# terminusdb-labs/parallel-hnsw

Measured on AMD Instinct MI355X. Metric: queries/sec at recall@10≥0.95 on 1M×768 f32, higher is better.
Workload: dtype f32

## Files before the change

### parallel_hnsw_amd/csrc/api.hip

```cpp
#include <hip/hip_runtime.h>

#include <algorithm>
#include <atomic>
#include <cmath>
#include <cstdarg>
#include <cstdio>
#include <cstring>
#include <new>
#include <stdexcept>
#include <vector>

#include "exact_slices.h"
#include "phnsw_internal.h"

static thread_local std::string g_err;

void ph_set_error(const char *fmt, ...) {
  char buf[1024];
  va_list ap;
  va_start(ap, fmt);
  vsnprintf(buf, sizeof(buf), fmt, ap);
  va_end(ap);
  g_err = buf;
}
// ... 614 lines not shown
    a.collect_k = c.collect_k;
    a.collect_flags = c.collect_flags;
    a.collect_ids = c.out_ids;
    a.collect_d = c.out_d;
    a.out_ids = nullptr;
    a.out_d = nullptr;
    a.filter_flags = 0u;
  }
}

uint32_t ph_default_ovf_cap(uint32_t ef) {
  if (const char *e = getenv("PHNSW_OVF_CAP"))
    if (atoi(e) > 0) return (uint32_t)atoi(e);
  return std::max<uint32_t>(8192u, ef * 64u);
}
static uint32_t default_ovf_cap(uint32_t ef) { return ph_default_ovf_cap(ef); }

static uint64_t two_launch_min() {
  const char *e = getenv("PHNSW_TWO_LAUNCH_MIN");
  return (e && atoll(e) > 0) ? (uint64_t)atoll(e) : (uint64_t)PH_TWO_LAUNCH_MIN;
}
static std::atomic<uint64_t> g_two_launch_count{0};
extern "C" uint64_t phnsw_debug_two_launch_count(void) { return g_two_launch_count.load(); }
extern "C" uint32_t phnsw_debug_last_search_chunks(const phnsw_index *ix) { return ix ? ix->ws[ix->ws_last].n_chunks : 0; }

extern "C" int phnsw_stream_create_beside(int device, void *other_stream, void **out_stream) try {
  if (!out_stream) {
    ph_set_error("phnsw_stream_create_beside: out_stream is NULL");
    return PHNSW_E_INVALID;
  }
  PH_HIP(hipSetDevice(device));
  hipStream_t st = nullptr;
  int rc = ph_stream_beside((hipStream_t)other_stream, &st);
  if (rc) return rc;
  *out_stream = (void *)st;
  return 0;
} catch (...) { return ph_caught(); }

static int attach_probes(phnsw_index *mix, const PhSearchCall &c, PhSearchArgs &a) {
  (void)mix, (void)c, (void)a;
#ifdef PH_CELL_PROBE
  {
    static unsigned long long *probe_dev = nullptr;
    if (!probe_dev) {
      PH_HIP(hipMalloc(&probe_dev, 12 * sizeof(unsigned long long)));
      PH_HIP(hipMemset(probe_dev, 0, 12 * sizeof(unsigned long long)));
// ... 89 lines not shown
  if (split) {
    g_two_launch_count++;
    rc = ph_workspace_order_ensure(ws, a.nq);
    for (uint32_t l = first_big; l < a.n_layers && !rc; l++)
      rc = ph_layer_anchor_pos(ix->store, mix->layers[l - 1]);
    if (rc) return rc;
    if (a.collect_k) {
      const size_t need = (size_t)nq * a.ef * 4u;
      if (ws.park_ids_bytes < need) {
        if (ws.park_ids) PH_HIP(hipFree(ws.park_ids));
        ws.park_ids = nullptr, ws.park_ids_bytes = 0;
        PH_HIP(hipMalloc(&ws.park_ids, need));
        ws.park_ids_bytes = need;
      }
      if (ws.park_d_bytes < need) {
        if (ws.park_d) PH_HIP(hipFree(ws.park_d));
        ws.park_d = nullptr, ws.park_d_bytes = 0;
        PH_HIP(hipMalloc(&ws.park_d, need));
        ws.park_d_bytes = need;
      }
      a.out_ids = ws.park_ids;
      a.out_d = ws.park_d;
    }
  }
  rc = attach_probes(mix, c, a);
  if (rc) return rc;
  rc = ph_search_begin(ws, stream);
  if (rc) return rc;
  bool kept_table = false;
  if (c.hint && T && !split) {
    rc = ph_build_table_prepare(mix, ws, a, *c.hint, T, stream, &kept_table);
    if (rc) return rc;
  }
  const uint64_t tmax = (T && !kept_table) ? ph_tiny_max_positions(ix, a.n_layers, a.ef) : 0;
  const uint64_t chunk = (tmax && nq > tmax) ? tmax : nq;
  for (uint64_t c0 = 0; c0 < nq; c0 += chunk) {
    PhSearchArgs b = a;
    const uint64_t cnt = std::min<uint64_t>(chunk, nq - c0);
    const bool last_chunk = c0 + cnt == nq;
    b.nq = (uint32_t)cnt;
    if (b.order) {
      b.order += c0;
    } else if (c0) {
      const uint32_t ostride = out_stride ? out_stride : b.ef;
      if (b.queries) b.queries += c0 * c.ldq;
      if (b.qids) b.qids += c0;
      if (b.exclude) b.exclude += c0;
      if (b.filter) b.filter += c0 * b.filter_stride;
      if (b.label_want) b.label_want += c0;
      if (b.out_ids) b.out_ids += c0 * ostride, b.out_d += c0 * ostride;
      if (b.collect_k) b.collect_ids += c0 * b.collect_k, b.collect_d += c0 * b.collect_k;
      b.out_len += c0;
      if (b.out_stats) b.out_stats += 2 * c0;
      b.status += c0;
      if (b.out_hit) b.out_hit += c0;
      b.first_node += (uint32_t)c0;
    }
    ws.n_chunks = (uint32_t)(c0 / chunk) + 1;
    PH_HIP(hipEventRecord(ws.evc, stream));
    if (c0) PH_HIP(hipMemsetAsync(ws.dtotals, 0, sizeof(unsigned long long) * 3 * PH_MAX_DISPATCH, stream));
    if (!kept_table) {
      rc = ph_tiny_prepare(ix, ws, b, T, stream);
      if (rc) return rc;
    }
    ws.d_tiny = b.tiny_layers != 0;
    PH_HIP(hipEventRecord(ws.evd[0], stream));
    if (!split) {
      b.launch_totals = ws.dtotals;
      b.launch_tab = ws.dtotals + 2 * PH_MAX_DISPATCH;
      rc = ph_search_launch(ix, ws, b, stream, last_chunk);
      if (rc) return rc;
      PH_HIP(hipEventRecord(ws.evd[1], stream));
      ws.n_dispatch = 1;
      ws.d_lo[0] = knn_mode ? b.n_layers - 1 : 0;
      ws.d_hi[0] = b.n_layers;
      continue;
    }
    const uint32_t Td = b.tiny_layers;
    const bool dense_first = Td && Td < b.n_layers && b.nq >= PH_DENSE_SPLIT_MIN && !getenv("PHNSW_NO_DENSE_SPLIT");
    if (dense_first) b.dense_flag = ws.tiny_member + b.tiny_n;
    uint32_t di = 0;
    uint32_t *const out_hit_final = b.out_hit;
    const uint32_t first_hi = dense_first ? Td : first_big;
    for (uint32_t lo = 0, hi = first_hi; lo < b.n_layers; lo = hi, hi = (lo == Td && dense_first && first_big > Td) ? first_big : hi + 1) {
      PhSearchArgs p = b;
// ... 649 lines not shown
```

### parallel_hnsw_amd/csrc/bruteforce.hip

```cpp
#include <hip/hip_runtime.h>

#include <algorithm>
#include <vector>

#include "phnsw_device.h"

typedef float f32x16 __attribute__((ext_vector_type(16)));

#define BF_TM 128
#define BF_TN 128
#define BF_TK 32
#define BF_LD 132

__global__ __launch_bounds__(256) void ph_gemm_nt_mfma_kernel(const float *__restrict__ Q, uint32_t ldq, uint32_t nq,
                                                              const float *__restrict__ B, uint32_t ldb, uint32_t nb,
                                                              uint32_t K, float *__restrict__ C, uint64_t ldc) {
  __shared__ float Qs[BF_TK][BF_LD];
  __shared__ float Bs[BF_TK][BF_LD];
  const uint32_t t = threadIdx.x, lane = t & 63, w = t >> 6;
  const uint32_t wm = w >> 1, wn = w & 1;
  const uint32_t q0 = blockIdx.y * BF_TM, b0 = blockIdx.x * BF_TN;
  f32x16 acc[2][2];
#pragma unroll
  for (int i = 0; i < 2; i++)
#pragma unroll
// ... 250 lines not shown
    }
    __syncthreads();
    if (t == 0) {
      float b = -PH_FMAX;
      uint32_t i = PH_EMPTY32;
      for (int k = 0; k < 16; k++)
        if (widx[k] != PH_EMPTY32 && (i == PH_EMPTY32 || wbest[k] > b || (wbest[k] == b && widx[k] < i))) {
          b = wbest[k];
          i = widx[k];
        }
      cur_s = i;
      seen[i] = 1;
      rank[i] = step;
    }
    __syncthreads();
  }
}

__global__ void ph_rank_of_cell_kernel(uint32_t *pos, uint32_t n, const uint32_t *rank) {
  uint32_t i = blockIdx.x * blockDim.x + threadIdx.x;
  if (i < n) pos[i] = rank[pos[i]];
}

static int ph_store_anchors(phnsw_store *s) {
  if (s->anchors) return 0;
  uint32_t amax = 4096u;
  if (const char *e = getenv("PHNSW_ANCHORS")) amax = atoi(e) >= 64 ? (uint32_t)atoi(e) : amax;
  const uint32_t A = (uint32_t)std::min<uint64_t>(amax, std::max<uint64_t>(s->n / 16u, 1u)), ld = s->ld;
  const uint64_t stride = s->n / A;
  float *anchors = nullptr, *gram = nullptr;
  uint32_t *rank = nullptr, *ids = nullptr;
  std::vector<uint32_t> h(A);
  for (uint32_t a = 0; a < A; a++) h[a] = (uint32_t)(a * stride);
  hipError_t e = hipMalloc(&anchors, (size_t)A * ld * 4);
  if (e == hipSuccess) e = hipMalloc(&gram, (size_t)A * A * 4);
  if (e == hipSuccess) e = hipMalloc(&rank, (size_t)A * 4);
  if (e == hipSuccess) e = hipMalloc(&ids, (size_t)A * 4);
  if (e == hipSuccess) e = hipMemcpy(ids, h.data(), (size_t)A * 4, hipMemcpyHostToDevice);
  if (e == hipSuccess) {
    if (ph_store_converted(s))
      (void)ph_converted_gather_rows(s, ids, 0, A, anchors);
    else
      hipLaunchKernelGGL(ph_gather_rows_f32_kernel, dim3((A + 3) / 4), dim3(256), 0, 0, s->rows, ld, ids, 1u, A, anchors);
    dim3 grid((A + BF_TN - 1) / BF_TN, (A + BF_TM - 1) / BF_TM);
    hipLaunchKernelGGL(ph_gemm_nt_mfma_kernel, grid, dim3(256), 0, 0, anchors, ld, A, anchors, ld, A, ld, gram, (uint64_t)A);
    hipLaunchKernelGGL(ph_anchor_chain_kernel, dim3(1), dim3(1024), (A + 32) * 4, 0, gram, A, rank);
    e = hipGetLastError();
    if (e == hipSuccess) e = hipDeviceSynchronize();
  }
  if (gram) hipFree(gram);
  if (ids) hipFree(ids);
  if (e != hipSuccess) {
    if (anchors) hipFree(anchors);
    if (rank) hipFree(rank);
    return ph_hip_fail(e, "store cells (anchors)", __FILE__, __LINE__);
  }
  s->anchors = anchors;
  s->anchor_rank = rank;
  s->n_anchors = A;
  return 0;
}

void ph_store_anchors_free(phnsw_store *s) {
  if (s->anchors) hipFree(s->anchors);
  if (s->anchor_rank) hipFree(s->anchor_rank);
  s->anchors = nullptr;
  s->anchor_rank = nullptr;
}

bool ph_layer_wants_cells(const phnsw_store *s, uint32_t n_nodes) {
  return n_nodes >= PH_POS_MIN && (ph_store_f32(s) || ph_store_converted(s)) && s->n >= 65536 && s->metric != PHNSW_METRIC_L2 && !getenv("PHNSW_NO_LOCALITY");
}

int ph_layer_cells_range(const phnsw_store *cs, const PhLayerHost &L, uint32_t first, uint32_t count, uint32_t *out_pos) {
  phnsw_store *s = const_cast<phnsw_store *>(cs);
  if (count == 0) return 0;
  int rc = ph_store_anchors(s);
  if (rc) return rc;
  const uint32_t A = s->n_anchors, ld = s->ld;
  const uint32_t QC = 65536;
  float *qrows = nullptr, *scores = nullptr;
  hipError_t e = hipMalloc(&scores, (size_t)std::min(QC, count) * A * 4);
  if (e == hipSuccess && (!L.identity || ph_store_converted(s))) e = hipMalloc(&qrows, (size_t)std::min(QC, count) * ld * 4);
  if (e == hipSuccess) {
    for (uint32_t at = 0; at < count; at += QC) {
      const uint32_t cnt = std::min(QC, count - at);
      const float *Q = ph_store_f32(s) ? s->rows + (uint64_t)(first + at) * ld : nullptr;
      if (ph_store_converted(s)) {
        (void)ph_converted_gather_rows(s, L.identity ? nullptr : L.nodes + first + at, first + at, cnt, qrows);
        Q = qrows;
      } else if (!L.identity) {
        hipLaunchKernelGGL(ph_gather_rows_f32_kernel, dim3((cnt + 3) / 4), dim3(256), 0, 0, s->rows, ld, L.nodes + first + at,
                           1u, cnt, qrows);
        Q = qrows;
      }
      dim3 grid((A + BF_TN - 1) / BF_TN, (cnt + BF_TM - 1) / BF_TM);
      hipLaunchKernelGGL(ph_gemm_nt_mfma_kernel, grid, dim3(256), 0, 0, Q, ld, cnt, s->anchors, ld, A,
                         std::min<uint32_t>(ld, 256u), scores, (uint64_t)A);
      hipLaunchKernelGGL(ph_argmax_rows_kernel, dim3(std::min<uint32_t>(cnt, 256u * 16u)), dim3(64), 0, 0, scores,
                         (uint64_t)A, A, cnt, out_pos + at);
    }
    hipLaunchKernelGGL(ph_rank_of_cell_kernel, dim3((count + 255) / 256), dim3(256), 0, 0, out_pos, count, s->anchor_rank);
    e = hipGetLastError();
    if (e == hipSuccess) e = hipDeviceSynchronize();
  }
  if (e != hipSuccess) rc = ph_hip_fail(e, "layer cells (anchor GEMM)", __FILE__, __LINE__);
  if (qrows) hipFree(qrows);
  if (scores) hipFree(scores);
  return rc;
}

int ph_layer_anchor_pos(const phnsw_store *cs, PhLayerHost &L) {
  const uint32_t n = L.n_nodes;
  if (L.pos || !ph_layer_wants_cells(cs, n)) return 0;
  hipError_t e = hipMalloc(&L.pos, (size_t)n * 4);
  if (e != hipSuccess) return ph_hip_fail(e, "layer cells", __FILE__, __LINE__);
  int rc = ph_layer_cells_range(cs, L, 0, n, L.pos);
  if (rc) {
    hipFree(L.pos);
    L.pos = nullptr;
  }
  return rc;
}

extern "C" float phnsw_bruteforce_last_gemm_ms(void) { return g_bf_gemm_ms; }

extern "C" int phnsw_bruteforce_topk(const phnsw_store *s, const float *queries, uint64_t nq, uint32_t k,
                                     uint64_t *out_ids, float *out_d) try {
  if (int rc = ph_search_only_unsupported(s, "phnsw_bruteforce_topk")) return rc;
  if (!s || !queries || !out_ids || !out_d || nq == 0) {
    ph_set_error("phnsw_bruteforce_topk: invalid argument");
    return PHNSW_E_INVALID;
  }
  PH_HIP(hipSetDevice(s->device));
  float *qd = nullptr, *od = nullptr;
  uint32_t *oid = nullptr;
  hipError_t e = hipMalloc(&qd, (size_t)nq * s->ld * 4);
  if (e == hipSuccess && s->ld != s->dim) e = hipMemset(qd, 0, (size_t)nq * s->ld * 4);
  if (e == hipSuccess)
    e = hipMemcpy2D(qd, (size_t)s->ld * 4, queries, (size_t)s->dim * 4, (size_t)s->dim * 4, nq, hipMemcpyHostToDevice);
  if (e == hipSuccess) e = hipMalloc(&oid, (size_t)nq * k * 4);
  if (e == hipSuccess) e = hipMalloc(&od, (size_t)nq * k * 4);
  int rc = e == hipSuccess ? 0 : ph_hip_fail(e, "bruteforce staging", __FILE__, __LINE__);
  if (!rc) rc = phnsw_bruteforce_topk_device(s, qd, s->ld, nq, k, oid, od, nullptr);
  if (!rc) {
    std::vector<uint32_t> h((size_t)nq * k);
// ... 13 lines not shown
```

### parallel_hnsw_amd/csrc/build.hip

```cpp
#include <hip/hip_runtime.h>

#include <algorithm>
#include <cmath>
#include <cstdio>
#include <cstdlib>
#include <cstring>
#include <numeric>
#include <vector>

#include "phnsw_device.h"

int ph_sort_u32_host(uint32_t *keys, uint32_t n);
int ph_exclusive_scan_u32(const uint32_t *cnt, uint32_t n_plus_1, uint32_t *start, hipStream_t st);


template <typename T>
struct DevBuf {
  T *p = nullptr;
  size_t n = 0;
  int alloc(size_t count) {
    n = count;
    hipError_t e = ph_pool_alloc((void **)&p, std::max<size_t>(count, 1) * sizeof(T));
    if (e != hipSuccess) {
      p = nullptr;
// ... 1136 lines not shown
      }
      nodes[o++] = vecs[b++];
    }
  }
  std::vector<uint32_t> nb((size_t)n_new * W, PH_EMPTY32);
  std::vector<float> nd((size_t)n_new * W, PH_FMAX);
  for (uint32_t i = 0; i < n_old; i++)
    for (uint32_t k = 0; k < W; k++) {
      uint32_t x = old_nb[(size_t)i * W + k];
      nb[(size_t)old_map[i] * W + k] = x == PH_EMPTY32 ? PH_EMPTY32 : old_map[x];
      if (!old_d.empty()) nd[(size_t)old_map[i] * W + k] = old_d[(size_t)i * W + k];
    }
  PhLayerHost NL;
  PH_TRY(ph_layer_upload(ix, nodes.data(), nb.data(), n_new, W, &NL));
  if (!old_d.empty()) {
    hipError_t e = hipMalloc(&NL.nbr_dist, nd.size() * 4);
    if (e == hipSuccess) e = hipMemcpy(NL.nbr_dist, nd.data(), nd.size() * 4, hipMemcpyHostToDevice);
    if (e != hipSuccess) {
      ph_layer_free(NL);
      return ph_hip_fail(e, "extend_layer upload", __FILE__, __LINE__);
    }
  }
  if (L.pos) {
    std::vector<uint32_t> op(n_old), np(n_new, PH_EMPTY32);
    PH_HIP(hipMemcpy(op.data(), L.pos, (size_t)n_old * 4, hipMemcpyDeviceToHost));
    for (uint32_t i = 0; i < n_old; i++) np[old_map[i]] = op[i];
    uint32_t next = n_old;
    for (uint32_t i = 0; i < n_new; i++)
      if (np[i] == PH_EMPTY32) np[i] = next++;
    hipError_t e = hipMalloc(&NL.pos, (size_t)n_new * 4);
    if (e == hipSuccess) e = hipMemcpy(NL.pos, np.data(), (size_t)n_new * 4, hipMemcpyHostToDevice);
    if (e != hipSuccess) {
      ph_layer_free(NL);
      return ph_hip_fail(e, "extend_layer positions", __FILE__, __LINE__);
    }
  }
  ph_layer_free(L);
  ix->layers[lft] = NL;
  return 0;
}

__global__ void ph_gather_rows_kernel(const uint32_t *neighbors, uint32_t W, const uint32_t *which, uint32_t cnt,
                                      uint32_t *out) {
  uint64_t i = (uint64_t)blockIdx.x * blockDim.x + threadIdx.x;
  if (i >= (uint64_t)cnt * W) return;
  out[i] = neighbors[(size_t)which[i / W] * W + (i % W)];
}

static int filter_promotion_candidates_impl(phnsw_index *ix, uint32_t lft, const std::vector<uint32_t> &vecs,
                                            const phnsw_search_params *sp, std::vector<uint32_t> &sel) {
  sel.clear();
  if (lft == 0) return 0;
// ... 479 lines not shown
```

### parallel_hnsw_amd/csrc/group.hip

```cpp
#include <hip/hip_runtime.h>
#include <hipcub/hipcub.hpp>

#include "phnsw_internal.h"

#include "phnsw_device.h"

__global__ void ph_group_keys_kernel(const uint32_t *init_ids, const float *init_d, const uint32_t *init_len,
                                     uint32_t K, uint32_t n, uint64_t *keys, uint32_t *vals) {
  uint32_t i = blockIdx.x * blockDim.x + threadIdx.x;
  if (i >= n) return;
  bool some = init_len[i] != 0;
  uint32_t key = some ? init_ids[(size_t)i * K] : PH_EMPTY32;
  float d = some ? init_d[(size_t)i * K] : 0.f;
  keys[i] = ((uint64_t)key << 32) | fkey(d);
  vals[i] = i;
}

__global__ void ph_group_bounds_kernel(const uint64_t *keys, uint32_t n, uint32_t *gstart, uint32_t *gsize) {
  uint32_t p = blockIdx.x * blockDim.x + threadIdx.x;
  if (p >= n) return;
  uint32_t k = (uint32_t)(keys[p] >> 32);
  uint32_t slot = k == PH_EMPTY32 ? n : k;
  if (p == 0 || (uint32_t)(keys[p - 1] >> 32) != k) gstart[slot] = p;
  atomicAdd(&gsize[slot], 1u);
// ... 41 lines not shown

int ph_order_by_keys_device(const uint32_t *keys, uint32_t n, uint32_t *order_out, hipStream_t st) {
  uint32_t *keys_out = nullptr, *vals_in = nullptr;
  void *tmp = nullptr;
  size_t tmp_bytes = 0;
  int rc = 0;
  hipError_t e = ph_pool_alloc((void **)&keys_out, (size_t)n * 4);
  if (e == hipSuccess) e = ph_pool_alloc((void **)&vals_in, (size_t)n * 4);
  if (e == hipSuccess)
    e = hipcub::DeviceRadixSort::SortPairs(nullptr, tmp_bytes, keys, keys_out, vals_in, order_out, (int)n, 0, 32, st);
  if (e == hipSuccess) e = ph_pool_alloc((void **)&tmp, std::max<size_t>(tmp_bytes, 16));
  if (e == hipSuccess) {
    hipLaunchKernelGGL(ph_iota_kernel, dim3((n + 255) / 256), dim3(256), 0, st, vals_in, n);
    e = hipcub::DeviceRadixSort::SortPairs(tmp, tmp_bytes, keys, keys_out, vals_in, order_out, (int)n, 0, 32, st);
    if (e == hipSuccess) e = hipStreamSynchronize(st);
  }
  if (e != hipSuccess) rc = ph_hip_fail(e, "query order (radix sort)", __FILE__, __LINE__);
  if (keys_out) ph_pool_free(keys_out);
  if (vals_in) ph_pool_free(vals_in);
  if (tmp) ph_pool_free(tmp);
  return rc;
}

int ph_exclusive_scan_u32(const uint32_t *cnt, uint32_t n_plus_1, uint32_t *start, hipStream_t st) {
  void *tmp = nullptr;
  size_t tmp_bytes = 0;
  hipError_t e = hipcub::DeviceScan::ExclusiveSum(nullptr, tmp_bytes, cnt, start, (int)n_plus_1, st);
  if (e == hipSuccess) e = ph_pool_alloc(&tmp, std::max<size_t>(tmp_bytes, 16));
  if (e == hipSuccess) e = hipcub::DeviceScan::ExclusiveSum(tmp, tmp_bytes, cnt, start, (int)n_plus_1, st);
  if (tmp) ph_pool_free(tmp);
  if (e != hipSuccess) return ph_hip_fail(e, "prefix sum", __FILE__, __LINE__);
  return 0;
}

int ph_sort_u32_host(uint32_t *keys, uint32_t n) {
  uint32_t *in = nullptr, *out = nullptr;
  void *tmp = nullptr;
  size_t tmp_bytes = 0;
  int rc = 0;
  hipError_t e = ph_pool_alloc((void **)&in, (size_t)n * 4);
  if (e == hipSuccess) e = ph_pool_alloc((void **)&out, (size_t)n * 4);
  if (e == hipSuccess) e = hipcub::DeviceRadixSort::SortKeys(nullptr, tmp_bytes, in, out, (int)n, 0, 32, (hipStream_t)0);
  if (e == hipSuccess) e = ph_pool_alloc(&tmp, std::max<size_t>(tmp_bytes, 16));
  if (e == hipSuccess) e = hipMemcpy(in, keys, (size_t)n * 4, hipMemcpyHostToDevice);
  if (e == hipSuccess) e = hipcub::DeviceRadixSort::SortKeys(tmp, tmp_bytes, in, out, (int)n, 0, 32, (hipStream_t)0);
  if (e == hipSuccess) e = hipMemcpy(keys, out, (size_t)n * 4, hipMemcpyDeviceToHost);
  if (e != hipSuccess) rc = ph_hip_fail(e, "node list sort", __FILE__, __LINE__);
  if (in) ph_pool_free(in);
  if (out) ph_pool_free(out);
  if (tmp) ph_pool_free(tmp);
  return rc;
}

void ph_workspace_order_free(PhWorkspace &ws) {
  if (ws.okey) hipFree(ws.okey);
  if (ws.okey_sorted) hipFree(ws.okey_sorted);
  if (ws.oiota) hipFree(ws.oiota);
  if (ws.oorder) hipFree(ws.oorder);
  if (ws.sort_tmp) hipFree(ws.sort_tmp);
  ws.okey = ws.okey_sorted = ws.oiota = ws.oorder = nullptr;
  ws.sort_tmp = nullptr;
  ws.sort_tmp_bytes = 0;
  ws.order_cap = 0;
}

int ph_workspace_order_ensure(PhWorkspace &ws, uint32_t nq) {
  if (ws.order_cap >= nq) return 0;
  ph_workspace_order_free(ws);
  uint32_t cap = std::max<uint32_t>(nq, 65536u);
  PH_HIP(hipMalloc(&ws.okey, (size_t)cap * 4));
  PH_HIP(hipMalloc(&ws.okey_sorted, (size_t)cap * 4));
  PH_HIP(hipMalloc(&ws.oiota, (size_t)cap * 4));
  PH_HIP(hipMalloc(&ws.oorder, (size_t)cap * 4));
  size_t bytes = 0;
  PH_HIP(hipcub::DeviceRadixSort::SortPairs(nullptr, bytes, ws.okey, ws.okey_sorted, ws.oiota, ws.oorder, (int)cap, 0, 32,
                                            (hipStream_t)0));
  ws.sort_tmp_bytes = std::max<size_t>(bytes, 16);
  PH_HIP(hipMalloc(&ws.sort_tmp, ws.sort_tmp_bytes));
  hipLaunchKernelGGL(ph_iota_kernel, dim3((cap + 255) / 256), dim3(256), 0, 0, ws.oiota, cap);
  PH_HIP(hipDeviceSynchronize());
  ws.order_cap = cap;
  return 0;
// ... 9 lines not shown
```

### parallel_hnsw_amd/csrc/phnsw_internal.h

```cpp
#pragma once
#include <hip/hip_runtime.h>
#include <stdint.h>
#include <stdlib.h>

#include <mutex>
#include <string>
#include <vector>

#include "../../include/phnsw.h"

#define PH_EMPTY32 0xFFFFFFFFu
#define PH_FMAX 3.4028234663852886e38f
#define PH_MAX_LAYERS 24
#define PH_WAVE 64
#define PH_MAX_DISPATCH 24
#define PH_DENSE_SPLIT_MIN 2048u
#define PH_TINY_MAX_NODES 8192u
#define PH_TINY_LDS_NODES 1024u
#define PH_TINY_MAX_LAYERS 8

void ph_set_error(const char *fmt, ...);
int ph_caught() noexcept;
int ph_hip_fail(hipError_t e, const char *what, const char *file, int line);
#define PH_HIP(x)                                                       \
// ... 55 lines not shown
  const uint16_t *codes16;
  const float *codebook;
  uint32_t m, ksub, dsub;
  uint32_t table_f16;
};

struct phnsw_store {
  int device = 0;
  int kind = PH_ROWS_F32;
  float *rows = nullptr;
  uint8_t *codes = nullptr;
  uint16_t *codes16 = nullptr;
  phnsw_store *centroid_store = nullptr;
  phnsw_index *centroid_index = nullptr;
  phnsw_search_params quantized_search = {0, 0, 0};
  float *codebook = nullptr;
  uint32_t pq_m = 0, pq_ksub = 0, pq_dsub = 0;
  uint32_t pq_table_f16 = 0;
  void *packed = nullptr;
  uint32_t packed_stride = 0;
  float *anchors = nullptr;
  uint32_t *anchor_rank = nullptr;
  uint32_t n_anchors = 0;
  bool owns_rows = true;
  uint64_t n = 0;
  uint32_t dim = 0, ld = 0;
  int metric = 0;
  int refcount = 1;
};

struct PhTinyPrepKey {
  bool valid = false;
  uint64_t nodes_epoch = 0;
  uint32_t T = 0, tn = 0;
  const void *nodes[PH_TINY_MAX_LAYERS] = {}, *nbrs[PH_TINY_MAX_LAYERS] = {}, *vec2node = nullptr;
  uint32_t n[PH_TINY_MAX_LAYERS] = {}, W[PH_TINY_MAX_LAYERS] = {};
  uint64_t links[PH_TINY_MAX_LAYERS] = {};
};
struct PhTinyPackKey {
  bool valid = false;
  uint64_t nodes_epoch = 0;
  const void *vecs = nullptr, *tnodes = nullptr;
  uint32_t ld = 0, tn = 0, nv = 0;
};

struct PhWorkspace {
  uint32_t *visited = nullptr;
  uint64_t visited_words = 0;
  uint2 *ovf = nullptr;
  uint32_t ovf_cap = 0;
  uint32_t n_slots = 0;
  uint32_t *counter = nullptr;
  hipEvent_t ev0 = nullptr, ev1 = nullptr;
  hipEvent_t evc = nullptr;
  bool timed = false;
  void *pq_tables = nullptr;
  size_t pq_tables_bytes = 0;
  uint32_t *okey = nullptr, *okey_sorted = nullptr, *oiota = nullptr, *oorder = nullptr;
  void *sort_tmp = nullptr;
  size_t sort_tmp_bytes = 0;
  uint32_t order_cap = 0;
  float *tiny_d = nullptr;
  size_t tiny_d_bytes = 0;
  uint32_t *tiny_nbr = nullptr;
  size_t tiny_nbr_bytes = 0;
  uint32_t *tiny_member = nullptr;
  size_t tiny_member_bytes = 0;
  float4 *tiny_pq = nullptr, *tiny_pn = nullptr;
  size_t tiny_pq_bytes = 0, tiny_pn_bytes = 0;
  PhTinyPrepKey tiny_prep_key;
  PhTinyPackKey tiny_pack_key;
  int tiny_table_g = 0;
  uint32_t tiny_last_npos = 0, tiny_last_tn = 0, tiny_last_stride = 0;
  uint2 *dense_ovf = nullptr;
  size_t dense_ovf_bytes = 0;
  uint32_t *ovf_s = nullptr;
  size_t ovf_s_cap = 0;
  uint32_t *park_ids = nullptr;
  float *park_d = nullptr;
  size_t park_ids_bytes = 0, park_d_bytes = 0;
  hipEvent_t evd[PH_MAX_DISPATCH + 1] = {};
  unsigned long long *dtotals = nullptr;
  uint32_t n_dispatch = 0;
  uint32_t n_chunks = 0;
// ... 125 lines not shown
  const uint32_t *probe_pos;
  unsigned long long *probe_out;
#endif
#ifdef PH_VISITED_PROBE
  unsigned long long *vprobe_out;
#endif
  uint32_t vis_slots, vis_limit, vis_off;
  const uint32_t *order;
  uint32_t seg;
  uint32_t *out_hit;
  uint32_t *out_index;
  uint32_t *ovf_s;
  uint32_t tiny_layers, tiny_n, tiny_stride;
  const float *tiny_d;
  const uint32_t *tiny_nbr;
  const uint32_t *tiny_member;
  uint32_t tiny_rows, tiny_row_first;
  const uint32_t *tiny_row_map;
  uint32_t tiny_off[PH_TINY_MAX_LAYERS];
  const uint32_t *label_of, *label_want;
  uint32_t collect_k, collect_flags;
  uint32_t *collect_ids;
  float *collect_d;
};

uint32_t ph_default_ovf_cap(uint32_t ef);
hipError_t ph_timed_malloc(void **p, size_t bytes);
hipError_t ph_timed_free(void *p);
#ifndef PH_RAW_ALLOC
#define hipMalloc(p, n) ph_timed_malloc((void **)(p), (n))
#define hipFree(p) ph_timed_free((void *)(p))
#endif
static inline long long env_ll(const char *name) {
  const char *e = getenv(name);
  return e ? atoll(e) : 0;
}
static inline uint32_t grid1(uint64_t items) {
  const uint64_t blocks = (items + 255u) / 256u;
  return (uint32_t)(blocks < (1u << 16) ? blocks : (1u << 16));
}
int ph_stream_beside(hipStream_t other, hipStream_t *io);
hipError_t ph_pool_alloc(void **p, size_t bytes);
void ph_pool_free(void *p);
void ph_pool_trim(void);
void ph_layer_free(PhLayerHost &l);
void ph_pending_free(phnsw_index *ix);
// ... 119 lines not shown
  const float *queries;
  uint32_t ldq;
  const uint32_t *qids, *exclude, *want;
  uint64_t nq;
  uint32_t k;
  uint32_t *out_ids;
  float *out_d;
  uint32_t *out_len, *status;
  hipStream_t stream;
  const uint32_t *list;
};
int ph_labeled_device(const phnsw_index *ix, const phnsw_labels *lb, const PhLabeledCall &c);
int ph_labels_fresh(const phnsw_index *ix, const phnsw_labels *lb, const char *call);
int ph_labeled_check(const phnsw_index *ix, const phnsw_labels *lb, uint64_t k, const char *call);
const uint32_t *ph_labels_column(const phnsw_labels *lb);
int ph_labels_count(const phnsw_labels *lb, const uint32_t *want_dev, uint64_t nq, uint32_t *out_count_dev, hipStream_t stream);
void ph_auto_free(phnsw_index *ix);
void ph_dense_free(phnsw_index *ix);
int ph_dense_check(const phnsw_index *ix, uint64_t k, const char *call);
void ph_grouped_free(phnsw_index *ix);
int ph_exact_check(const phnsw_index *ix, uint64_t k, const char *call);
#define PH_ORDER_MIN 16384u
#define PH_POS_MIN 256u
#define PH_SPLIT_BYTES (4ull << 20)
static inline bool ph_layer_own_launch(uint64_t n_nodes, uint32_t row_bytes) {
  const char *e = getenv("PHNSW_SPLIT_BYTES");
  const uint64_t limit = (e && atoll(e) > 0) ? (uint64_t)atoll(e) : (uint64_t)PH_SPLIT_BYTES;
  return n_nodes * (uint64_t)row_bytes > limit;
}
int ph_layer_anchor_pos(const phnsw_store *s, PhLayerHost &L);
bool ph_layer_wants_cells(const phnsw_store *s, uint32_t n_nodes);
int ph_layer_cells_range(const phnsw_store *s, const PhLayerHost &L, uint32_t first, uint32_t count, uint32_t *out_pos);
void ph_store_anchors_free(phnsw_store *s);
int ph_order_by_keys_device(const uint32_t *keys, uint32_t n, uint32_t *order_out, hipStream_t st);
int ph_layer_range_order(PhLayerHost &L, uint32_t first, uint32_t count, const uint32_t **out);

static inline bool ph_store_converted(const phnsw_store *s) { return ph_rows_converted(s->kind); }
static inline bool ph_store_f32(const phnsw_store *s) { return s->kind == PH_ROWS_F32; }
static inline bool ph_store_pq(const phnsw_store *s) { return s->kind == PH_ROWS_PQ; }
static inline bool ph_store_pq_shared(const phnsw_store *s) { return s->kind == PH_ROWS_PQ_SHARED; }
int ph_converted_gather_rows(const phnsw_store *s, const uint32_t *ids_dev, uint32_t first, uint32_t cnt, float *out_dev);
int ph_converted_store_read(const phnsw_store *s, uint64_t first, uint64_t count, float *out);

int ph_tiny_prepare(const phnsw_index *ix, PhWorkspace &ws, PhSearchArgs &a, uint32_t max_layers, hipStream_t stream);
int ph_build_table_prepare(phnsw_index *ix, PhWorkspace &ws, PhSearchArgs &a, const PhRowHint &h, uint32_t T,
                           hipStream_t stream, bool *used);
void ph_build_table_free(phnsw_index *ix);
size_t ph_tiny_lds_bytes(const PhSearchArgs &a);
bool ph_tiny_matrix_cores(const phnsw_index *ix);
uint32_t ph_tiny_layer_count(const phnsw_index *ix, uint32_t n_layers, uint32_t ef);
uint64_t ph_tiny_max_positions(const phnsw_index *ix, uint32_t n_layers, uint32_t ef);
void ph_tiny_free(PhWorkspace &ws);
int ph_tiny_table_chunk(const phnsw_index *ix, PhWorkspace &ws, const float *queries, uint32_t ldq, const uint32_t *qids,
                        const uint32_t *order, uint32_t npos, const uint32_t *tnodes, uint32_t tn, float *D, hipStream_t stream,
                        bool *kept);

int ph_search_begin(PhWorkspace &ws, hipStream_t stream);
int ph_search_launch(const phnsw_index *ix, PhWorkspace &ws, PhSearchArgs &a, hipStream_t stream, bool mark_end = true);
// ... 97 lines not shown
```

### parallel_hnsw_amd/csrc/search_kernels.h

```cpp
#pragma once
#include <hip/hip_runtime.h>

#include <algorithm>
#include <cstdio>
#include <cstdlib>
#include <cstring>

#include "phnsw_internal.h"

#include "phnsw_device.h"

#ifdef PH_HOP_PROFILE
#define PH_TICK(k)                                   \
  {                                                  \
    asm volatile("s_waitcnt vmcnt(0) lgkmcnt(0)");   \
    const uint64_t t_now = wall_clock64();           \
    tprof[k] += t_now - t_last;                      \
    t_last = t_now;                                  \
  }
#else
#define PH_TICK(k)
#endif

template <bool BIG>
// ... 96 lines not shown
        if (lane == 0) p = atomicAdd(a.counter + seg_cur * 16u, 1u);
        p = rfl32(p);
        const uint32_t base = seg_cur * a.seg;
        const uint32_t len = base >= a.nq ? 0u : min(a.seg, a.nq - base);
        if (p < len) {
          qpos = base + p;
          q = a.order[qpos];
          break;
        }
        seg_cur = (seg_cur + 1u) & 7u;
        if (++seg_done == 8u) {
          q = PH_EMPTY32;
          break;
        }
      }
      if (q == PH_EMPTY32) break;
    }

    const uint32_t last_layer = a.n_layers - 1;
    const uint32_t layer_hi = a.layer_hi ? a.layer_hi : a.n_layers;
    if (layer_lo && a.status[q] != ST_OK) continue;
    const uint32_t qnode = (BIG && a.knn_nodes) ? a.knn_nodes[q] : a.first_node + q;
    uint32_t qvec = a.knn_mode ? a.layers[last_layer].nodes[qnode] : (a.qids ? a.qids[q] : 0u);
    uint64_t trow = qpos;
    if (a.tiny_rows) trow = (uint64_t)((a.tiny_row_map ? a.tiny_row_map[qvec] : qvec) - a.tiny_row_first);
    Dist dist;
    if (a.queries && !a.knn_mode)
      dist.prepare_raw(a.dist, a.queries + (uint64_t)q * a.ldq, dist_lds, lane);
    else
      dist.prepare_stored(a.dist, qvec, dist_lds, lane);
    const uint32_t excl = a.exclude ? a.exclude[q] : PH_EMPTY32;
    const uint32_t *const allow = FM == PH_FM_BITMAP ? a.filter + (uint64_t)q * a.filter_stride : nullptr;
    const uint32_t want = FM == PH_FM_LABEL ? rfl32(a.label_want[q]) : PHNSW_LABEL_NONE;
    auto passes = [&](uint32_t v) -> bool {
      if constexpr (FM == PH_FM_BITMAP) {
        return (allow[v >> 5] >> (v & 31)) & 1u;
      } else if constexpr (FM == PH_FM_LABEL) {
        const uint32_t lbl = a.label_of[v];
        return lbl == want && lbl != PHNSW_LABEL_NONE;
      } else {
        return true;
      }
    };
    uint64_t kq = KEY_NONE;
    uint32_t klen = 0;
    auto collect = [&](uint64_t ckey) -> bool {
      const uint32_t kk = a.collect_k;
// ... 859 lines not shown
```

### parallel_hnsw_amd/csrc/tiny.hip

```cpp
#include <hip/hip_runtime.h>

#include <algorithm>
#include <cstdlib>
#include <cstring>

#include "phnsw_device.h"

struct PhTinyPrepArgs {
  PhLayerDev layers[PH_TINY_MAX_LAYERS];
  uint32_t T, tiny_n;
  uint32_t off[PH_TINY_MAX_LAYERS];
  uint32_t *nbr;
  uint32_t *member;
};

__global__ void ph_tiny_prep_kernel(PhTinyPrepArgs p) {
  const uint32_t l = blockIdx.y;
  const PhLayerDev L = p.layers[l], TL = p.layers[p.T - 1];
  for (uint32_t i = blockIdx.x * blockDim.x + threadIdx.x; i < L.n_nodes; i += gridDim.x * blockDim.x) {
    const uint32_t vid = L.nodes[i];
    const uint32_t t = TL.vec2node ? TL.vec2node[vid] : vid;
    if (t >= p.tiny_n) {
      p.member[p.tiny_n] = 1u;
      continue;
// ... 777 lines not shown
  if (getenv("PHNSW_VERBOSE")) {
    if (ws.tiny_table_g)
      fprintf(stderr, "[phnsw] dense table: %u positions x %u nodes on the matrix cores, G = %d (%s), graph %s, node operand %s\n",
              npos, tn, ws.tiny_table_g, beside ? "beside the other workspace's launch" : "alone",
              prep_kept ? "kept" : "prepared", pack_kept ? "kept" : "packed");
    else
      fprintf(stderr, "[phnsw] dense table: %u positions x %u nodes on the vector units, graph %s\n", npos, tn,
              prep_kept ? "kept" : "prepared");
  }
  ws.tiny_last_npos = npos;
  ws.tiny_last_tn = tn;
  ws.tiny_last_stride = stride;
  a.tiny_layers = T;
  a.tiny_n = tn;
  a.tiny_lds_nodes = PH_TINY_LDS_NODES;
  a.tiny_stride = stride;
  a.tiny_d = ws.tiny_d;
  a.tiny_nbr = ws.tiny_nbr;
  a.tiny_member = ws.tiny_member;
  return 0;
}


void ph_build_table_free(phnsw_index *ix) {
  for (PhBuildTable &b : ix->bt)
    if (b.D) ph_timed_free(b.D);
  ix->bt.clear();
  for (auto &sp : ix->bt_spare) ph_timed_free(sp.first);
  ix->bt_spare.clear();
}
static void build_table_drop(phnsw_index *ix, PhBuildTable &b) {
  if (b.D) ix->bt_spare.emplace_back(b.D, b.cap);
  b.D = nullptr;
  b.bytes = b.cap = 0;
  b.lo = b.hi = b.lo_alloc = b.hi_alloc = 0;
}
static void build_table_recycle(phnsw_index *ix) {
  for (PhBuildTable &b : ix->bt) build_table_drop(ix, b);
  ix->bt.clear();
}
static float *build_table_buffer(phnsw_index *ix, size_t bytes, size_t *cap) {
  int best = -1;
  for (size_t i = 0; i < ix->bt_spare.size(); i++)
    if (ix->bt_spare[i].second >= bytes && ix->bt_spare[i].second <= 2 * bytes &&
        (best < 0 || ix->bt_spare[i].second < ix->bt_spare[(size_t)best].second))
      best = (int)i;
// ... 116 lines not shown
```

Measured before the change: 1.077 million.

## Order queries by dense-table cell for locality and refine anchors by means

After the dense upper-layer table is computed, each query is assigned the majority cell among its four nearest table nodes. Queries are then counting-sorted by cell so that neighbouring workgroups traverse similar graph regions and share cache. Anchors are also refined with one k-means-style mean step, and the anchor argmax now uses the full dimension instead of 256 dims. The cost is extra kernels per search (top-4, histogram, scan, scatter) and a heavier one-time anchor build.

```diff
diff --git a/parallel_hnsw_amd/csrc/api.hip b/parallel_hnsw_amd/csrc/api.hip
--- a/parallel_hnsw_amd/csrc/api.hip
+++ b/parallel_hnsw_amd/csrc/api.hip
@@ -660,6 +660,8 @@
 }
 static std::atomic<uint64_t> g_two_launch_count{0};
 extern "C" uint64_t phnsw_debug_two_launch_count(void) { return g_two_launch_count.load(); }
+static std::atomic<uint64_t> g_table_order_count{0};
+extern "C" uint64_t phnsw_debug_table_order_count(void) { return g_table_order_count.load(); }
 extern "C" uint32_t phnsw_debug_last_search_chunks(const phnsw_index *ix) { return ix ? ix->ws[ix->ws_last].n_chunks : 0; }
 
 extern "C" int phnsw_stream_create_beside(int device, void *other_stream, void **out_stream) try {
@@ -795,6 +797,16 @@
       a.out_ids = ws.park_ids;
       a.out_d = ws.park_d;
     }
+  }
+  const uint32_t *table_pos = nullptr;
+  const char *const table_order_env = getenv("PHNSW_TABLE_ORDER");
+  if (T && !split && !a.order && !knn_mode && !out_stride && !out_index && !c.hint && !c.out_hit && !a.filter && !a.label_of &&
+      !a.collect_k && nq >= PH_TABLE_ORDER_MIN && !getenv("PHNSW_NO_LOCALITY") && !(table_order_env && table_order_env[0] == '0')) {
+    PhLayerHost &TL = mix->layers[T - 1];
+    rc = ph_layer_anchor_pos(ix->store, TL);
+    if (!rc && TL.pos) rc = ph_workspace_order_ensure(ws, a.nq);
+    if (rc) return rc;
+    table_pos = TL.pos;
   }
   rc = attach_probes(mix, c, a);
   if (rc) return rc;
@@ -834,6 +846,10 @@
     if (c0) PH_HIP(hipMemsetAsync(ws.dtotals, 0, sizeof(unsigned long long) * 3 * PH_MAX_DISPATCH, stream));
     if (!kept_table) {
       rc = ph_tiny_prepare(ix, ws, b, T, stream);
+      if (!rc && table_pos && b.tiny_layers == T) {
+        rc = ph_tiny_table_order(ws, b, table_pos, ix->store->n_anchors, stream);
+        if (!rc && b.table_by_query) g_table_order_count++;
+      }
       if (rc) return rc;
     }
     ws.d_tiny = b.tiny_layers != 0;
diff --git a/parallel_hnsw_amd/csrc/bruteforce.hip b/parallel_hnsw_amd/csrc/bruteforce.hip
--- a/parallel_hnsw_amd/csrc/bruteforce.hip
+++ b/parallel_hnsw_amd/csrc/bruteforce.hip
@@ -1,6 +1,7 @@
 #include <hip/hip_runtime.h>
 
 #include <algorithm>
+#include <cstring>
 #include <vector>
 
 #include "phnsw_device.h"
@@ -297,12 +298,95 @@
   if (i < n) pos[i] = rank[pos[i]];
 }
 
+__global__ __launch_bounds__(256) void ph_anchor_mean_kernel(const float *__restrict__ rows, uint64_t row_stride, uint32_t ld,
+                                                             const uint32_t *__restrict__ start,
+                                                             const uint32_t *__restrict__ members, uint32_t A,
+                                                             const float *__restrict__ old, float *__restrict__ out) {
+  __shared__ float wsum[4];
+  const uint32_t a = blockIdx.x, t = threadIdx.x;
+  if (a >= A) return;
+  const uint32_t first = start[a], cnt = start[a + 1u] - first;
+  float ss = 0.f;
+  for (uint32_t j = t; j < ld; j += 256u) {
+    float acc = 0.f;
+    for (uint32_t i = 0; i < cnt; i++) acc += rows[(uint64_t)members[first + i] * row_stride + j];
+    out[(uint64_t)a * ld + j] = acc;
+    ss += acc * acc;
+  }
+#pragma unroll
+  for (int sft = 32; sft >= 1; sft >>= 1) ss += __shfl_xor(ss, sft);
+  if ((t & 63u) == 0) wsum[t >> 6] = ss;
+  __syncthreads();
+  const float norm = sqrtf(((wsum[0] + wsum[1]) + wsum[2]) + wsum[3]);
+  const bool keep = !(norm > 0.f) || !(norm < PH_FMAX);
+  for (uint32_t j = t; j < ld; j += 256u)
+    out[(uint64_t)a * ld + j] = keep ? old[(uint64_t)a * ld + j] : out[(uint64_t)a * ld + j] / norm;
+}
+
+#define PH_CELL_SAMPLE 262144u
+
+static int ph_refine_anchors(const phnsw_store *s, uint32_t A, const float *raw, float *refined) {
+  const uint32_t ld = s->ld, m = (uint32_t)std::min<uint64_t>(s->n, PH_CELL_SAMPLE);
+  const uint64_t step = s->n / m;
+  const uint32_t QC = 65536;
+  float *samp = nullptr, *scores = nullptr;
+  uint32_t *cell = nullptr, *start = nullptr, *members = nullptr, *ids = nullptr;
+  const float *base = s->rows;
+  uint64_t row_stride = step * ld;
+  int rc = 0;
+  hipError_t e = hipMalloc(&scores, (size_t)std::min(QC, m) * A * 4);
+  if (e == hipSuccess) e = hipMalloc(&cell, (size_t)m * 4);
+  if (e == hipSuccess) e = hipMalloc(&start, ((size_t)A + 1u) * 4);
+  if (e == hipSuccess) e = hipMalloc(&members, (size_t)m * 4);
+  if (e == hipSuccess && (ph_store_converted(s) || row_stride > 0xFFFFFFFCull)) {
+    std::vector<uint32_t> h(m);
+    for (uint32_t i = 0; i < m; i++) h[i] = (uint32_t)(i * step);
+    e = hipMalloc(&samp, (size_t)m * ld * 4);
+    if (e == hipSuccess) e = hipMalloc(&ids, (size_t)m * 4);
+    if (e == hipSuccess) e = hipMemcpy(ids, h.data(), (size_t)m * 4, hipMemcpyHostToDevice);
+    if (e == hipSuccess) {
+      if (ph_store_converted(s))
+        rc = ph_converted_gather_rows(s, ids, 0, m, samp);
+      else
+        hipLaunchKernelGGL(ph_gather_rows_f32_kernel, dim3((m + 3) / 4), dim3(256), 0, 0, s->rows, ld, ids, 1u, m, samp);
+    }
+    base = samp;
+    row_stride = ld;
+  }
+  if (e == hipSuccess && !rc) {
+    for (uint32_t at = 0; at < m; at += QC) {
+      const uint32_t cnt = std::min(QC, m - at);
+      dim3 grid((A + BF_TN - 1) / BF_TN, (cnt + BF_TM - 1) / BF_TM);
+      hipLaunchKernelGGL(ph_gemm_nt_mfma_kernel, grid, dim3(256), 0, 0, base + (uint64_t)at * row_stride, (uint32_t)row_stride,
+                         cnt, raw, ld, A, ld, scores, (uint64_t)A);
+      hipLaunchKernelGGL(ph_argmax_rows_kernel, dim3(std::min<uint32_t>(cnt, 256u * 16u)), dim3(64), 0, 0, scores, (uint64_t)A,
+                         A, cnt, cell + at);
+    }
+    rc = ph_cell_order_device(cell, m, A, start, members, 0);
+    if (!rc) {
+      hipLaunchKernelGGL(ph_anchor_mean_kernel, dim3(A), dim3(256), 0, 0, base, row_stride, ld, start, members, A, raw, refined);
+      e = hipGetLastError();
+      if (e == hipSuccess) e = hipDeviceSynchronize();
+    }
+  }
+  if (e != hipSuccess) rc = ph_hip_fail(e, "store cells (anchor means)", __FILE__, __LINE__);
+  if (samp) hipFree(samp);
+  if (ids) hipFree(ids);
+  if (scores) hipFree(scores);
+  if (cell) hipFree(cell);
+  if (start) hipFree(start);
+  if (members) hipFree(members);
+  return rc;
+}
+
 static int ph_store_anchors(phnsw_store *s) {
   if (s->anchors) return 0;
   uint32_t amax = 4096u;
   if (const char *e = getenv("PHNSW_ANCHORS")) amax = atoi(e) >= 64 ? (uint32_t)atoi(e) : amax;
   const uint32_t A = (uint32_t)std::min<uint64_t>(amax, std::max<uint64_t>(s->n / 16u, 1u)), ld = s->ld;
   const uint64_t stride = s->n / A;
+  const char *const cells_env = getenv("PHNSW_CELLS");
+  const bool cells_raw = cells_env && !strcmp(cells_env, "raw");
   float *anchors = nullptr, *gram = nullptr;
   uint32_t *rank = nullptr, *ids = nullptr;
   std::vector<uint32_t> h(A);
@@ -317,6 +401,15 @@
       (void)ph_converted_gather_rows(s, ids, 0, A, anchors);
     else
       hipLaunchKernelGGL(ph_gather_rows_f32_kernel, dim3((A + 3) / 4), dim3(256), 0, 0, s->rows, ld, ids, 1u, A, anchors);
+    if (!cells_raw) {
+      float *refined = nullptr;
+      e = hipMalloc(&refined, (size_t)A * ld * 4);
+      if (e == hipSuccess && ph_refine_anchors(s, A, anchors, refined)) e = hipErrorUnknown;
+      if (e == hipSuccess) std::swap(anchors, refined);
+      if (refined) hipFree(refined);
+    }
+  }
+  if (e == hipSuccess) {
     dim3 grid((A + BF_TN - 1) / BF_TN, (A + BF_TM - 1) / BF_TM);
     hipLaunchKernelGGL(ph_gemm_nt_mfma_kernel, grid, dim3(256), 0, 0, anchors, ld, A, anchors, ld, A, ld, gram, (uint64_t)A);
     hipLaunchKernelGGL(ph_anchor_chain_kernel, dim3(1), dim3(1024), (A + 32) * 4, 0, gram, A, rank);
@@ -333,6 +426,7 @@
   s->anchors = anchors;
   s->anchor_rank = rank;
   s->n_anchors = A;
+  s->cells_raw = cells_raw;
   return 0;
 }
 
@@ -371,7 +465,7 @@
       }
       dim3 grid((A + BF_TN - 1) / BF_TN, (cnt + BF_TM - 1) / BF_TM);
       hipLaunchKernelGGL(ph_gemm_nt_mfma_kernel, grid, dim3(256), 0, 0, Q, ld, cnt, s->anchors, ld, A,
-                         std::min<uint32_t>(ld, 256u), scores, (uint64_t)A);
+                         s->cells_raw ? std::min<uint32_t>(ld, 256u) : ld, scores, (uint64_t)A);
       hipLaunchKernelGGL(ph_argmax_rows_kernel, dim3(std::min<uint32_t>(cnt, 256u * 16u)), dim3(64), 0, 0, scores,
                          (uint64_t)A, A, cnt, out_pos + at);
     }
@@ -397,6 +491,35 @@
   }
   return rc;
 }
+
+extern "C" int phnsw_debug_store_cells(phnsw_store *s, float *anchors_out, uint32_t *rank_out, uint32_t *n_anchors_out) try {
+  if (!s || !n_anchors_out || !(ph_store_f32(s) || ph_store_converted(s)) || s->n < 16 || s->metric == PHNSW_METRIC_L2) {
+    ph_set_error("phnsw_debug_store_cells: need an f32, f16 or i8 store with a dot-product metric");
+    return PHNSW_E_INVALID;
+  }
+  PH_HIP(hipSetDevice(s->device));
+  if (int rc = ph_store_anchors(s)) return rc;
+  *n_anchors_out = s->n_anchors;
+  if (anchors_out) PH_HIP(hipMemcpy(anchors_out, s->anchors, (size_t)s->n_anchors * s->ld * 4, hipMemcpyDeviceToHost));
+  if (rank_out) PH_HIP(hipMemcpy(rank_out, s->anchor_rank, (size_t)s->n_anchors * 4, hipMemcpyDeviceToHost));
+  return 0;
+} catch (...) { return ph_caught(); }
+
+extern "C" int phnsw_debug_layer_cells(phnsw_index *ix, uint32_t lft, uint32_t *pos_out) try {
+  if (!ix || !pos_out || lft >= ix->layers.size()) {
+    ph_set_error("phnsw_debug_layer_cells: invalid argument");
+    return PHNSW_E_INVALID;
+  }
+  PH_HIP(hipSetDevice(ix->store->device));
+  PhLayerHost &L = ix->layers[lft];
+  if (int rc = ph_layer_anchor_pos(ix->store, L)) return rc;
+  if (!L.pos) {
+    ph_set_error("phnsw_debug_layer_cells: layer %u carries no cells", lft);
+    return PHNSW_E_UNSUPPORTED;
+  }
+  PH_HIP(hipMemcpy(pos_out, L.pos, (size_t)L.n_nodes * 4, hipMemcpyDeviceToHost));
+  return 0;
+} catch (...) { return ph_caught(); }
 
 extern "C" float phnsw_bruteforce_last_gemm_ms(void) { return g_bf_gemm_ms; }
 
diff --git a/parallel_hnsw_amd/csrc/build.hip b/parallel_hnsw_amd/csrc/build.hip
--- a/parallel_hnsw_amd/csrc/build.hip
+++ b/parallel_hnsw_amd/csrc/build.hip
@@ -1182,12 +1182,27 @@
     }
   }
   if (L.pos) {
-    std::vector<uint32_t> op(n_old), np(n_new, PH_EMPTY32);
+    std::vector<uint32_t> op(n_old), np(n_new, PH_EMPTY32), fresh_at, fresh;
     PH_HIP(hipMemcpy(op.data(), L.pos, (size_t)n_old * 4, hipMemcpyDeviceToHost));
     for (uint32_t i = 0; i < n_old; i++) np[old_map[i]] = op[i];
-    uint32_t next = n_old;
     for (uint32_t i = 0; i < n_new; i++)
-      if (np[i] == PH_EMPTY32) np[i] = next++;
+      if (np[i] == PH_EMPTY32) fresh_at.push_back(i), fresh.push_back(nodes[i]);
+    int crc = 0;
+    if (!fresh.empty()) {
+      DevBuf<uint32_t> fnodes, fpos;
+      crc = fnodes.alloc(fresh.size());
+      if (!crc) crc = fpos.alloc(fresh.size());
+      if (!crc && hipMemcpy(fnodes.p, fresh.data(), fresh.size() * 4, hipMemcpyHostToDevice) != hipSuccess) crc = PHNSW_E_HIP;
+      PhLayerHost F;
+      F.nodes = fnodes.p, F.n_nodes = (uint32_t)fresh.size(), F.identity = false;
+      if (!crc) crc = ph_layer_cells_range(ix->store, F, 0, F.n_nodes, fpos.p);
+      if (!crc && hipMemcpy(fresh.data(), fpos.p, fresh.size() * 4, hipMemcpyDeviceToHost) != hipSuccess) crc = PHNSW_E_HIP;
+      for (size_t k = 0; k < fresh.size() && !crc; k++) np[fresh_at[k]] = fresh[k];
+    }
+    if (crc) {
+      ph_layer_free(NL);
+      return crc;
+    }
     hipError_t e = hipMalloc(&NL.pos, (size_t)n_new * 4);
     if (e == hipSuccess) e = hipMemcpy(NL.pos, np.data(), (size_t)n_new * 4, hipMemcpyHostToDevice);
     if (e != hipSuccess) {
diff --git a/parallel_hnsw_amd/csrc/group.hip b/parallel_hnsw_amd/csrc/group.hip
--- a/parallel_hnsw_amd/csrc/group.hip
+++ b/parallel_hnsw_amd/csrc/group.hip
@@ -87,6 +87,94 @@
   return rc;
 }
 
+static __device__ __forceinline__ uint32_t cell_of_key(uint32_t key, uint32_t bins) { return key < bins ? key : bins - 1u; }
+
+__global__ void ph_cell_hist_kernel(const uint32_t *keys, uint32_t n, uint32_t bins, uint32_t *cnt) {
+  for (uint32_t i = blockIdx.x * blockDim.x + threadIdx.x; i < n; i += gridDim.x * blockDim.x)
+    atomicAdd(&cnt[cell_of_key(keys[i], bins)], 1u);
+}
+
+__global__ __launch_bounds__(1024) void ph_cell_prefix_kernel(uint32_t *cnt, uint32_t bins) {
+  __shared__ uint32_t part[1024];
+  const uint32_t t = threadIdx.x, per = (bins + 1u + 1023u) / 1024u;
+  const uint32_t lo = min(t * per, bins + 1u), hi = min(lo + per, bins + 1u);
+  uint32_t sum = 0;
+  for (uint32_t i = lo; i < hi; i++) sum += cnt[i];
+  part[t] = sum;
+  __syncthreads();
+  for (uint32_t d = 1; d < 1024u; d <<= 1) {
+    const uint32_t v = t >= d ? part[t - d] : 0u;
+    __syncthreads();
+    part[t] += v;
+    __syncthreads();
+  }
+  uint32_t run = part[t] - sum;
+  for (uint32_t i = lo; i < hi; i++) {
+    const uint32_t c = cnt[i];
+    cnt[i] = run;
+    run += c;
+  }
+}
+
+__global__ __launch_bounds__(64) void ph_cell_scatter_kernel(const uint32_t *__restrict__ keys, uint32_t n, uint32_t bins,
+                                                             const uint32_t *__restrict__ start, uint32_t *__restrict__ order) {
+  const uint32_t lane = threadIdx.x;
+  const uint64_t lt = lanemask_lt(lane);
+  for (uint32_t b = blockIdx.x; b < bins; b += gridDim.x) {
+    const uint32_t first = start[b], want = start[b + 1u] - first;
+    uint32_t have = 0;
+    for (uint32_t base = 0; base < n && have < want; base += 256u) {
+      uint32_t k[4];
+#pragma unroll
+      for (int j = 0; j < 4; j++) {
+        const uint32_t i = base + 64u * j + lane;
+        k[j] = i < n ? cell_of_key(keys[i], bins) : PH_EMPTY32;
+      }
+#pragma unroll
+      for (int j = 0; j < 4; j++) {
+        const bool mine = k[j] == b;
+        const uint64_t m = __ballot(mine);
+        const uint32_t at = first + have + (uint32_t)__popcll(m & lt);
+        if (mine && at < n) order[at] = base + 64u * j + lane;
+        have += (uint32_t)__popcll(m);
+      }
+    }
+  }
+}
+
+int ph_cell_order_device(const uint32_t *keys, uint32_t n, uint32_t bins, uint32_t *start, uint32_t *order_out, hipStream_t st) {
+  if (n == 0 || bins == 0) return 0;
+  PH_HIP(hipMemsetAsync(start, 0, ((size_t)bins + 1u) * 4u, st));
+  hipLaunchKernelGGL(ph_cell_hist_kernel, dim3(grid1(n)), dim3(256), 0, st, keys, n, bins, start);
+  hipLaunchKernelGGL(ph_cell_prefix_kernel, dim3(1), dim3(1024), 0, st, start, bins);
+  hipLaunchKernelGGL(ph_cell_scatter_kernel, dim3(std::min<uint32_t>(bins, 1u << 16)), dim3(64), 0, st, keys, n, bins, start,
+                     order_out);
+  PH_HIP(hipGetLastError());
+  return 0;
+}
+
+extern "C" int phnsw_debug_cell_order(const uint32_t *keys, uint32_t n, uint32_t bins, uint32_t *order_out) try {
+  if (!keys || !order_out || n == 0 || bins == 0 || bins > (1u << 24)) {
+    ph_set_error("phnsw_debug_cell_order: invalid argument");
+    return PHNSW_E_INVALID;
+  }
+  uint32_t *k = nullptr, *start = nullptr, *order = nullptr;
+  hipError_t e = ph_pool_alloc((void **)&k, (size_t)n * 4);
+  if (e == hipSuccess) e = ph_pool_alloc((void **)&start, ((size_t)bins + 1u) * 4);
+  if (e == hipSuccess) e = ph_pool_alloc((void **)&order, (size_t)n * 4);
+  if (e == hipSuccess) e = hipMemcpy(k, keys, (size_t)n * 4, hipMemcpyHostToDevice);
+  if (e == hipSuccess) e = hipMemset(order, 0xFF, (size_t)n * 4);
+  int rc = e == hipSuccess ? ph_cell_order_device(k, n, bins, start, order, 0) : ph_hip_fail(e, "cell order staging", __FILE__, __LINE__);
+  if (!rc) {
+    e = hipMemcpy(order_out, order, (size_t)n * 4, hipMemcpyDeviceToHost);
+    if (e != hipSuccess) rc = ph_hip_fail(e, "cell order readback", __FILE__, __LINE__);
+  }
+  if (k) ph_pool_free(k);
+  if (start) ph_pool_free(start);
+  if (order) ph_pool_free(order);
+  return rc;
+} catch (...) { return ph_caught(); }
+
 int ph_exclusive_scan_u32(const uint32_t *cnt, uint32_t n_plus_1, uint32_t *start, hipStream_t st) {
   void *tmp = nullptr;
   size_t tmp_bytes = 0;
@@ -123,6 +211,9 @@
   if (ws.oiota) hipFree(ws.oiota);
   if (ws.oorder) hipFree(ws.oorder);
   if (ws.sort_tmp) hipFree(ws.sort_tmp);
+  if (ws.ocell) hipFree(ws.ocell);
+  ws.ocell = nullptr;
+  ws.ocell_cap = 0;
   ws.okey = ws.okey_sorted = ws.oiota = ws.oorder = nullptr;
   ws.sort_tmp = nullptr;
   ws.sort_tmp_bytes = 0;
diff --git a/parallel_hnsw_amd/csrc/phnsw_internal.h b/parallel_hnsw_amd/csrc/phnsw_internal.h
--- a/parallel_hnsw_amd/csrc/phnsw_internal.h
+++ b/parallel_hnsw_amd/csrc/phnsw_internal.h
@@ -101,6 +101,7 @@
   float *anchors = nullptr;
   uint32_t *anchor_rank = nullptr;
   uint32_t n_anchors = 0;
+  bool cells_raw = false;
   bool owns_rows = true;
   uint64_t n = 0;
   uint32_t dim = 0, ld = 0;
@@ -139,6 +140,8 @@
   void *sort_tmp = nullptr;
   size_t sort_tmp_bytes = 0;
   uint32_t order_cap = 0;
+  uint32_t *ocell = nullptr;
+  uint32_t ocell_cap = 0;
   float *tiny_d = nullptr;
   size_t tiny_d_bytes = 0;
   uint32_t *tiny_nbr = nullptr;
@@ -310,6 +313,7 @@
   uint32_t collect_k, collect_flags;
   uint32_t *collect_ids;
   float *collect_d;
+  uint32_t table_by_query;
 };
 
 uint32_t ph_default_ovf_cap(uint32_t ef);
@@ -475,6 +479,7 @@
 int ph_exact_check(const phnsw_index *ix, uint64_t k, const char *call);
 #define PH_ORDER_MIN 16384u
 #define PH_POS_MIN 256u
+#define PH_TABLE_ORDER_MIN 2048u
 #define PH_SPLIT_BYTES (4ull << 20)
 static inline bool ph_layer_own_launch(uint64_t n_nodes, uint32_t row_bytes) {
   const char *e = getenv("PHNSW_SPLIT_BYTES");
@@ -487,6 +492,8 @@
 void ph_store_anchors_free(phnsw_store *s);
 int ph_order_by_keys_device(const uint32_t *keys, uint32_t n, uint32_t *order_out, hipStream_t st);
 int ph_layer_range_order(PhLayerHost &L, uint32_t first, uint32_t count, const uint32_t **out);
+int ph_cell_order_device(const uint32_t *keys, uint32_t n, uint32_t bins, uint32_t *start, uint32_t *order_out, hipStream_t st);
+int ph_tiny_table_order(PhWorkspace &ws, PhSearchArgs &b, const uint32_t *pos, uint32_t bins, hipStream_t stream);
 
 static inline bool ph_store_converted(const phnsw_store *s) { return ph_rows_converted(s->kind); }
 static inline bool ph_store_f32(const phnsw_store *s) { return s->kind == PH_ROWS_F32; }
diff --git a/parallel_hnsw_amd/csrc/search_kernels.h b/parallel_hnsw_amd/csrc/search_kernels.h
--- a/parallel_hnsw_amd/csrc/search_kernels.h
+++ b/parallel_hnsw_amd/csrc/search_kernels.h
@@ -142,7 +142,7 @@
     if (layer_lo && a.status[q] != ST_OK) continue;
     const uint32_t qnode = (BIG && a.knn_nodes) ? a.knn_nodes[q] : a.first_node + q;
     uint32_t qvec = a.knn_mode ? a.layers[last_layer].nodes[qnode] : (a.qids ? a.qids[q] : 0u);
-    uint64_t trow = qpos;
+    uint64_t trow = a.table_by_query ? q : qpos;
     if (a.tiny_rows) trow = (uint64_t)((a.tiny_row_map ? a.tiny_row_map[qvec] : qvec) - a.tiny_row_first);
     Dist dist;
     if (a.queries && !a.knn_mode)
diff --git a/parallel_hnsw_amd/csrc/tiny.hip b/parallel_hnsw_amd/csrc/tiny.hip
--- a/parallel_hnsw_amd/csrc/tiny.hip
+++ b/parallel_hnsw_amd/csrc/tiny.hip
@@ -823,6 +823,68 @@
 }
 
 
+__global__ __launch_bounds__(64) void ph_tiny_row_cell_kernel(const float *__restrict__ D, uint32_t stride, uint32_t tn,
+                                                              uint32_t nq, const uint32_t *__restrict__ pos,
+                                                              uint32_t *__restrict__ key) {
+  const uint32_t lane = threadIdx.x;
+  for (uint32_t q = blockIdx.x; q < nq; q += gridDim.x) {
+    const float *row = D + (uint64_t)q * stride;
+    uint64_t top[4] = {KEY_NONE, KEY_NONE, KEY_NONE, KEY_NONE};
+    for (uint32_t t = lane; t < tn; t += 64) {
+      uint64_t k = mkkey(row[t], t);
+      if (k < top[3]) {
+#pragma unroll
+        for (int j = 0; j < 4; j++) {
+          const uint64_t lo = k < top[j] ? k : top[j], hi = k < top[j] ? top[j] : k;
+          top[j] = lo;
+          k = hi;
+        }
+      }
+    }
+    uint32_t cell[4], n = 0;
+#pragma unroll
+    for (int r = 0; r < 4; r++) {
+      uint64_t m = top[0];
+#pragma unroll
+      for (int s = 32; s >= 1; s >>= 1) {
+        const uint64_t o = __shfl_xor(m, s);
+        m = o < m ? o : m;
+      }
+      if (top[0] == m) top[0] = top[1], top[1] = top[2], top[2] = top[3], top[3] = KEY_NONE;
+      const uint32_t t = (uint32_t)m & IDM;
+      cell[r] = 0u;
+      if (m != KEY_NONE && t < tn) cell[r] = pos[t], n = r + 1;
+    }
+    uint32_t best = 0, best_cnt = 0;
+#pragma unroll
+    for (int i = 0; i < 4; i++) {
+      uint32_t cnt = 0;
+#pragma unroll
+      for (int j = 0; j < 4; j++) cnt += ((uint32_t)j < n && cell[j] == cell[i]) ? 1u : 0u;
+      if ((uint32_t)i < n && cnt > best_cnt) best = cell[i], best_cnt = cnt;
+    }
+    if (lane == 0) key[q] = best;
+  }
+}
+
+int ph_tiny_table_order(PhWorkspace &ws, PhSearchArgs &b, const uint32_t *pos, uint32_t bins, hipStream_t stream) {
+  if (!b.tiny_layers || b.tiny_rows || !pos || !bins || ws.order_cap < b.nq) return 0;
+  if (ws.ocell_cap < bins) {
+    if (ws.ocell) PH_HIP(hipFree(ws.ocell));
+    ws.ocell = nullptr, ws.ocell_cap = 0;
+    PH_HIP(hipMalloc(&ws.ocell, ((size_t)bins + 1u) * 4u));
+    ws.ocell_cap = bins;
+  }
+  hipLaunchKernelGGL(ph_tiny_row_cell_kernel, dim3(std::min<uint32_t>(b.nq, 1u << 16)), dim3(64), 0, stream, b.tiny_d,
+                     b.tiny_stride, b.tiny_n, b.nq, pos, ws.okey);
+  int rc = ph_cell_order_device(ws.okey, b.nq, bins, ws.ocell, ws.oorder, stream);
+  if (rc) return rc;
+  b.order = ws.oorder;
+  b.table_by_query = 1u;
+  return 0;
+}
+
+
 void ph_build_table_free(phnsw_index *ix) {
   for (PhBuildTable &b : ix->bt)
     if (b.D) ph_timed_free(b.D);
```

Result: faster. 1.211 million, median of 6 (+12.4%).
